# anovos/anovos

Measured on AMD Instinct MI355X. Metric: rows/sec (whole node) full analyzer+drift+transform, higher is better.
Workload: dtype fp32 data + fp64 accumulators; 1 GPU; model=anovos-full-pipeline, rows_per_gpu=125000000, n_cols=201, global_batch=125000000, parallelism=dp1

## Files before the change

### anovos_amd/ops/hip/anovos_kernels.hip

```cpp

#include <hip/hip_runtime.h>
#include <cfloat>
#include <cstdint>
#include <cmath>

#define THREADS 256
#define DEV_INLINE __device__ __forceinline__

typedef int nat_i4 __attribute__((ext_vector_type(4)));
typedef float nat_f4 __attribute__((ext_vector_type(4)));


#define NSTAT 9

struct MomAcc {
  double n, s1, s2, s3, s4, mn, mx, zn, nf;
};

DEV_INLINE void mom_add(MomAcc &a, double v, double shift) {
  if (!isnan(v)) {
    a.n += 1.0;
    double d = v - shift;
    a.s1 += d;
    double d2 = d * d;
    a.s2 += d2;
    a.s3 += d2 * d;
    a.s4 += d2 * d2;
    a.mn = fmin(a.mn, v);
    a.mx = fmax(a.mx, v);
    a.zn += (v == 0.0) ? 1.0 : 0.0;
    a.nf += (v != trunc(v)) ? 1.0 : 0.0;
  }
}

DEV_INLINE void mom_wave_reduce(MomAcc &a) {
  for (int off = 32; off > 0; off >>= 1) {
    a.n += __shfl_down(a.n, off);
    a.s1 += __shfl_down(a.s1, off);
    a.s2 += __shfl_down(a.s2, off);
    a.s3 += __shfl_down(a.s3, off);
    a.s4 += __shfl_down(a.s4, off);
    a.mn = fmin(a.mn, __shfl_down(a.mn, off));
    a.mx = fmax(a.mx, __shfl_down(a.mx, off));
    a.zn += __shfl_down(a.zn, off);
    a.nf += __shfl_down(a.nf, off);
  }
}

DEV_INLINE void mom_block_reduce_write(MomAcc &a, double *dst) {
  mom_wave_reduce(a);
  __shared__ double smw[(THREADS / 64) * NSTAT];
  const int wave = threadIdx.x >> 6;
  if ((threadIdx.x & 63) == 0) {
    double *m = &smw[wave * NSTAT];
    m[0] = a.n; m[1] = a.s1; m[2] = a.s2; m[3] = a.s3; m[4] = a.s4;
    m[5] = a.mn; m[6] = a.mx; m[7] = a.zn; m[8] = a.nf;
  }
  __syncthreads();
  if (threadIdx.x == 0) {
    MomAcc r{0, 0, 0, 0, 0, (double)INFINITY, -(double)INFINITY, 0, 0};
    for (int wv = 0; wv < THREADS / 64; ++wv) {
      double *m = &smw[wv * NSTAT];
      r.n += m[0]; r.s1 += m[1]; r.s2 += m[2]; r.s3 += m[3]; r.s4 += m[4];
      r.mn = fmin(r.mn, m[5]); r.mx = fmax(r.mx, m[6]);
      r.zn += m[7]; r.nf += m[8];
    }
    dst[0] = r.n; dst[1] = r.s1; dst[2] = r.s2; dst[3] = r.s3; dst[4] = r.s4;
    dst[5] = r.mn; dst[6] = r.mx; dst[7] = r.zn; dst[8] = r.nf;
  }
}

template <typename T>
__global__ __launch_bounds__(THREADS) void moments_partials_kernel(
    const T *const *cols, const int64_t *lens, const double *shifts, int nchunks,
    double *partials) {
  const int col = blockIdx.x / nchunks;
  const int chunk = blockIdx.x % nchunks;
  const T *__restrict__ x = cols[col];
  const int64_t n = lens[col];
  const double shift = shifts ? shifts[col] : 0.0;
  const int64_t per = (n + nchunks - 1) / nchunks;
  const int64_t s = (int64_t)chunk * per;
  const int64_t e = min(n, s + per);

  MomAcc a{0, 0, 0, 0, 0, (double)INFINITY, -(double)INFINITY, 0};

  if (sizeof(T) == 4) {
    const int64_t nv = (e - s) / 4;
    const float4 *xv = reinterpret_cast<const float4 *>(x + s);
    for (int64_t i = threadIdx.x; i < nv; i += THREADS) {
      float4 v = xv[i];
      mom_add(a, (double)v.x, shift);
      mom_add(a, (double)v.y, shift);
      mom_add(a, (double)v.z, shift);
      mom_add(a, (double)v.w, shift);
    }
    for (int64_t i = s + nv * 4 + threadIdx.x; i < e; i += THREADS) mom_add(a, (double)x[i], shift);
  } else {
    for (int64_t i = s + threadIdx.x; i < e; i += THREADS) mom_add(a, (double)x[i], shift);
  }

  mom_block_reduce_write(a, &partials[(int64_t)blockIdx.x * NSTAT]);
}

__global__ __launch_bounds__(THREADS) void moments_reduce_kernel(
    const double *partials, int nchunks, double *out) {
  const int col = blockIdx.x;
  MomAcc a{0, 0, 0, 0, 0, (double)INFINITY, -(double)INFINITY, 0, 0};
  for (int c = threadIdx.x; c < nchunks; c += THREADS) {
    const double *p = &partials[((int64_t)col * nchunks + c) * NSTAT];
    a.n += p[0]; a.s1 += p[1]; a.s2 += p[2]; a.s3 += p[3]; a.s4 += p[4];
    a.mn = fmin(a.mn, p[5]); a.mx = fmax(a.mx, p[6]); a.zn += p[7]; a.nf += p[8];
  }
  __shared__ double sm[THREADS * NSTAT];
  double *mine = &sm[threadIdx.x * NSTAT];
  mine[0] = a.n; mine[1] = a.s1; mine[2] = a.s2; mine[3] = a.s3;
  mine[4] = a.s4; mine[5] = a.mn; mine[6] = a.mx; mine[7] = a.zn; mine[8] = a.nf;
  __syncthreads();
  for (int stride = THREADS / 2; stride > 0; stride >>= 1) {
    if (threadIdx.x < stride) {
      double *other = &sm[(threadIdx.x + stride) * NSTAT];
      mine[0] += other[0]; mine[1] += other[1]; mine[2] += other[2];
      mine[3] += other[3]; mine[4] += other[4];
      mine[5] = fmin(mine[5], other[5]);
      mine[6] = fmax(mine[6], other[6]);
      mine[7] += other[7]; mine[8] += other[8];
    }
    __syncthreads();
  }
  if (threadIdx.x == 0) {
    double *o = &out[(int64_t)col * NSTAT];
    o[0] = sm[0]; o[1] = sm[1]; o[2] = sm[2]; o[3] = sm[3]; o[4] = sm[4];
    o[5] = (sm[0] > 0) ? sm[5] : nan("");
    o[6] = (sm[0] > 0) ? sm[6] : nan("");
    o[7] = sm[7]; o[8] = sm[8];
  }
}


template <typename T>
__global__ __launch_bounds__(THREADS) void hist_kernel(
    const T *const *cols, const int64_t *lens, const double *lo, const double *hi,
    int nbins, int nchunks, uint64_t *out ) {
  extern __shared__ uint32_t bins[];
  const int col = blockIdx.x / nchunks;
  const int chunk = blockIdx.x % nchunks;
  for (int b = threadIdx.x; b < nbins; b += THREADS) bins[b] = 0;
  __syncthreads();

  const T *__restrict__ x = cols[col];
  const int64_t n = lens[col];
  const int64_t per = (n + nchunks - 1) / nchunks;
  const int64_t s = (int64_t)chunk * per;
  const int64_t e = min(n, s + per);
  const double l = lo[col];
  const double h = hi[col];
  if (h > l) {
    const double scale = (double)nbins / (h - l);
    auto body = [&](double v) {
      if (!isnan(v)) {
        const double t = fmin(fmax((v - l) * scale, 0.0), (double)(nbins - 1));
        atomicAdd(&bins[(int)t], 1u);
      }
    };
    if (sizeof(T) == 4) {
      const int64_t nv = (e - s) / 4;
      const float4 *xv = reinterpret_cast<const float4 *>(x + s);
      for (int64_t i = threadIdx.x; i < nv; i += THREADS) {
        float4 v = xv[i];
        body((double)v.x);
        body((double)v.y);
        body((double)v.z);
        body((double)v.w);
      }
      for (int64_t i = s + nv * 4 + threadIdx.x; i < e; i += THREADS) body((double)x[i]);
    } else {
      for (int64_t i = s + threadIdx.x; i < e; i += THREADS) body((double)x[i]);
    }
  } else {
    for (int64_t i = s + threadIdx.x; i < e; i += THREADS) {
      double v = (double)x[i];
      if (!isnan(v)) atomicAdd(&bins[0], 1u);
    }
  }
  __syncthreads();
  uint64_t *g = &out[(int64_t)col * nbins];
  for (int b = threadIdx.x; b < nbins; b += THREADS)
    if (bins[b]) atomicAdd((unsigned long long *)&g[b], (unsigned long long)bins[b]);
}

template <typename T>
__global__ __launch_bounds__(THREADS) void bracket_hist_kernel(
    const T *const *cols, const int64_t *lens, const int64_t *colidx,
    const double *lo, const double *hi, int nbins, int nchunks, uint64_t *out) {
  extern __shared__ uint32_t bins[];
  const int bracket = blockIdx.x / nchunks;
  const int chunk = blockIdx.x % nchunks;
  for (int b = threadIdx.x; b < nbins; b += THREADS) bins[b] = 0;
  __syncthreads();
  const int col = (int)colidx[bracket];
  const T *__restrict__ x = cols[col];
  const int64_t n = lens[col];
  const int64_t per = (n + nchunks - 1) / nchunks;
  const int64_t s = (int64_t)chunk * per;
  const int64_t e = min(n, s + per);
  const double l = lo[bracket];
  const double h = hi[bracket];
  if (h > l) {
    const double scale = (double)nbins / (h - l);
    for (int64_t i = s + threadIdx.x; i < e; i += THREADS) {
      double v = (double)x[i];
      if (!isnan(v) && v >= l && v < h) {
        int b = (int)((v - l) * scale);
        b = max(0, min(nbins - 1, b));
        atomicAdd(&bins[b], 1u);
      }
    }
  }
  __syncthreads();
  uint64_t *g = &out[(int64_t)bracket * nbins];
  for (int b = threadIdx.x; b < nbins; b += THREADS)
    if (bins[b]) atomicAdd((unsigned long long *)&g[b], (unsigned long long)bins[b]);
}

#define RB_BINS 512
#define RB_MAXB 16

template <typename T>
__global__ __launch_bounds__(THREADS) void bracket_hist_grouped_kernel(
    const T *const *cols, const int64_t *lens, const int *bstart, int ncols,
    const double *lo, const double *hi, const double *p1lo,
    const double *p1scale, int p1bins, int nchunks, uint64_t *out) {
  __shared__ uint32_t bins[RB_MAXB * RB_BINS];
  extern __shared__ int16_t lut[];
  __shared__ double slo[RB_MAXB], sscale[RB_MAXB], shi[RB_MAXB];
  const int col = blockIdx.x / nchunks;
  const int chunk = blockIdx.x % nchunks;
  const int b0 = bstart[col];
  const int nb = bstart[col + 1] - b0;
  if (nb == 0) return;
  const double l1 = p1lo[col];
  const double sc1 = p1scale[col];
  for (int i = threadIdx.x; i < nb * RB_BINS; i += THREADS) bins[i] = 0;
  for (int i = threadIdx.x; i < p1bins; i += THREADS) lut[i] = -1;
  __syncthreads();
  if (threadIdx.x < nb) {
    const double bl = lo[b0 + threadIdx.x];
    const double bh = hi[b0 + threadIdx.x];
    slo[threadIdx.x] = bl;
    shi[threadIdx.x] = bh;
    double w = bh - bl;
    sscale[threadIdx.x] = (w > 0) ? (double)RB_BINS / w : 0.0;
    const double mid = (bl + bh) * 0.5;
    const int bin1 = (int)fmin(fmax((mid - l1) * sc1, 0.0), (double)(p1bins - 1));
// ... 245 lines not shown
}

__global__ __launch_bounds__(THREADS) void lut_apply_f32_kernel(
    const int32_t *const *cols, const int64_t *lens, const float *lutflat,
    const int64_t *lut_off, int nchunks, float *const *outs) {
  const int col = blockIdx.x / nchunks;
  const int chunk = blockIdx.x % nchunks;
  const int32_t *__restrict__ codes = cols[col];
  float *__restrict__ out = outs[col];
  const float *__restrict__ lut = &lutflat[lut_off[col]];
  const int64_t n = lens[col];
  const int64_t per = (n + nchunks - 1) / nchunks;
  const int64_t s = (int64_t)chunk * per;
  const int64_t e = min(n, s + per);
  const nat_i4 *__restrict__ cv = reinterpret_cast<const nat_i4 *>(codes + s);
  nat_f4 *__restrict__ ov = reinterpret_cast<nat_f4 *>(out + s);
  const int64_t nv = (e - s) / 4;
  for (int64_t i = threadIdx.x; i < nv; i += THREADS) {
    nat_i4 c = __builtin_nontemporal_load(&cv[i]);
    nat_f4 r;
    r.x = (c.x < 0) ? nanf("") : lut[c.x];
    r.y = (c.y < 0) ? nanf("") : lut[c.y];
    r.z = (c.z < 0) ? nanf("") : lut[c.z];
    r.w = (c.w < 0) ? nanf("") : lut[c.w];
    __builtin_nontemporal_store(r, &ov[i]);
  }
  for (int64_t j = s + nv * 4 + threadIdx.x; j < e; j += THREADS) {
    int c = codes[j];
    out[j] = (c < 0) ? nanf("") : lut[c];
  }
}

__global__ __launch_bounds__(THREADS) void lut_apply_i32_kernel(
    const int32_t *const *cols, const int64_t *lens, const int32_t *lutflat,
    const int64_t *lut_off, int nchunks, int32_t *const *outs) {
  const int col = blockIdx.x / nchunks;
  const int chunk = blockIdx.x % nchunks;
  const int32_t *__restrict__ codes = cols[col];
  int32_t *__restrict__ out = outs[col];
  const int32_t *__restrict__ lut = &lutflat[lut_off[col]];
  const int64_t n = lens[col];
  const int64_t per = (n + nchunks - 1) / nchunks;
  const int64_t s = (int64_t)chunk * per;
  const int64_t e = min(n, s + per);
  const nat_i4 *__restrict__ cv = reinterpret_cast<const nat_i4 *>(codes + s);
  nat_i4 *__restrict__ ov = reinterpret_cast<nat_i4 *>(out + s);
  const int64_t nv = (e - s) / 4;
  for (int64_t i = threadIdx.x; i < nv; i += THREADS) {
    nat_i4 c = __builtin_nontemporal_load(&cv[i]);
    nat_i4 r;
    r.x = (c.x < 0) ? -1 : lut[c.x];
    r.y = (c.y < 0) ? -1 : lut[c.y];
    r.z = (c.z < 0) ? -1 : lut[c.z];
    r.w = (c.w < 0) ? -1 : lut[c.w];
    __builtin_nontemporal_store(r, &ov[i]);
  }
  for (int64_t j = s + nv * 4 + threadIdx.x; j < e; j += THREADS) {
    int c = codes[j];
    out[j] = (c < 0) ? -1 : lut[c];
  }
}

__global__ __launch_bounds__(THREADS) void fill_code_kernel(
    const int32_t *const *cols, const int64_t *lens, const int32_t *fill,
    int nchunks, int32_t *const *outs) {
  const int col = blockIdx.x / nchunks;
  const int chunk = blockIdx.x % nchunks;
  const int32_t *__restrict__ x = cols[col];
  int32_t *__restrict__ out = outs[col];
  const int64_t n = lens[col];
  const int32_t fv = fill[col];
  const int64_t per = (n + nchunks - 1) / nchunks;
  const int64_t s = (int64_t)chunk * per;
  const int64_t e = min(n, s + per);
  const nat_i4 *__restrict__ xv = reinterpret_cast<const nat_i4 *>(x + s);
  nat_i4 *__restrict__ ov = reinterpret_cast<nat_i4 *>(out + s);
  const int64_t nv = (e - s) / 4;
  int64_t i = threadIdx.x;
  for (; i + THREADS < nv; i += 2 * THREADS) {
    nat_i4 a = __builtin_nontemporal_load(&xv[i]);
    nat_i4 b = __builtin_nontemporal_load(&xv[i + THREADS]);
    a.x = (a.x == -1) ? fv : a.x;
    a.y = (a.y == -1) ? fv : a.y;
    a.z = (a.z == -1) ? fv : a.z;
    a.w = (a.w == -1) ? fv : a.w;
    b.x = (b.x == -1) ? fv : b.x;
    b.y = (b.y == -1) ? fv : b.y;
    b.z = (b.z == -1) ? fv : b.z;
    b.w = (b.w == -1) ? fv : b.w;
    __builtin_nontemporal_store(a, &ov[i]);
    __builtin_nontemporal_store(b, &ov[i + THREADS]);
  }
  for (; i < nv; i += THREADS) {
    nat_i4 a = xv[i];
    a.x = (a.x == -1) ? fv : a.x;
    a.y = (a.y == -1) ? fv : a.y;
    a.z = (a.z == -1) ? fv : a.z;
    a.w = (a.w == -1) ? fv : a.w;
    ov[i] = a;
  }
  for (int64_t j = s + nv * 4 + threadIdx.x; j < e; j += THREADS) {
    int32_t c = x[j];
    out[j] = (c == -1) ? fv : c;
  }
}


__global__ __launch_bounds__(THREADS) void code_counts_kernel(
    const int32_t *codes, int64_t n, int size, int nchunks, uint64_t *out) {
  extern __shared__ uint32_t cnt[];
  const bool use_lds = (size <= 16384);
  if (use_lds) {
    for (int i = threadIdx.x; i < size; i += THREADS) cnt[i] = 0;
    __syncthreads();
  }
  const int chunk = blockIdx.x;
  const int64_t per = (n + nchunks - 1) / nchunks;
  const int64_t s = (int64_t)chunk * per;
  const int64_t e = min(n, s + per);
  if (use_lds) {
    for (int64_t i = s + threadIdx.x; i < e; i += THREADS) {
      int c = codes[i];
      if (c >= 0 && c < size) atomicAdd(&cnt[c], 1u);
    }
    __syncthreads();
    for (int i = threadIdx.x; i < size; i += THREADS)
      if (cnt[i]) atomicAdd((unsigned long long *)&out[i], (unsigned long long)cnt[i]);
  } else {
    for (int64_t i = s + threadIdx.x; i < e; i += THREADS) {
      int c = codes[i];
      if (c >= 0 && c < size) atomicAdd((unsigned long long *)&out[c], 1ull);
    }
  }
}


DEV_INLINE uint64_t splitmix64(uint64_t x) {
  x ^= x >> 30; x *= 0xBF58476D1CE4E5B9ull;
  x ^= x >> 27; x *= 0x94D049BB133111EBull;
  x ^= x >> 31;
  return x;
}

DEV_INLINE uint32_t fmix32(uint32_t x) {
  x ^= x >> 16;
  x *= 0x85EBCA6Bu;
  x ^= x >> 13;
  x *= 0xC2B2AE35u;
  x ^= x >> 16;
  return x;
}

template <typename T>
DEV_INLINE bool hll_hash(T v, int p, int &idx, int &rho) {
  if (sizeof(T) == 4) {
    float f = (float)v;
    if (isnan(f)) return false;
    uint32_t b32;
    memcpy(&b32, &f, 4);
    uint32_t h = fmix32(b32);
    idx = (int)(h >> (32 - p));
    uint32_t rem = h << p;
    rho = (rem == 0) ? (32 - p + 1) : (__clz((int)rem) + 1);
    if (rho > 32 - p + 1) rho = 32 - p + 1;
    return true;
  }
  double d = (double)v;
  if (isnan(d)) return false;
  uint64_t bits;
  memcpy(&bits, &d, 8);
  uint64_t h = splitmix64(bits);
  idx = (int)(h >> (64 - p));
  uint64_t rem = h << p;
  rho = (rem == 0) ? (64 - p + 1) : (__clzll((long long)rem) + 1);
  if (rho > 64 - p + 1) rho = 64 - p + 1;
  return true;
}

template <typename T>
__global__ __launch_bounds__(THREADS) void hll_kernel(
    const T *x, int64_t n, int p, int nchunks, int32_t *regs ) {
  extern __shared__ int32_t sreg[];
  const int m = 1 << p;
  for (int i = threadIdx.x; i < m; i += THREADS) sreg[i] = 0;
  __syncthreads();
  const int chunk = blockIdx.x;
  const int64_t per = (n + nchunks - 1) / nchunks;
  const int64_t s = (int64_t)chunk * per;
  const int64_t e = min(n, s + per);
  if (sizeof(T) == 4) {
    const float4 *xv = reinterpret_cast<const float4 *>(x + s);
    const int64_t nv = (e - s) / 4;
    for (int64_t i = threadIdx.x; i < nv; i += THREADS) {
      float4 v = xv[i];
      int idx, rho;
      if (hll_hash((T)v.x, p, idx, rho)) { if (sreg[idx] < rho) atomicMax(&sreg[idx], rho); }
      if (hll_hash((T)v.y, p, idx, rho)) { if (sreg[idx] < rho) atomicMax(&sreg[idx], rho); }
      if (hll_hash((T)v.z, p, idx, rho)) { if (sreg[idx] < rho) atomicMax(&sreg[idx], rho); }
      if (hll_hash((T)v.w, p, idx, rho)) { if (sreg[idx] < rho) atomicMax(&sreg[idx], rho); }
    }
    for (int64_t i = s + nv * 4 + threadIdx.x; i < e; i += THREADS) {
      int idx, rho;
      if (hll_hash(x[i], p, idx, rho)) { if (sreg[idx] < rho) atomicMax(&sreg[idx], rho); }
    }
  } else {
    for (int64_t i = s + threadIdx.x; i < e; i += THREADS) {
      int idx, rho;
      if (hll_hash(x[i], p, idx, rho)) { if (sreg[idx] < rho) atomicMax(&sreg[idx], rho); }
    }
  }
  __syncthreads();
  for (int i = threadIdx.x; i < m; i += THREADS)
    if (sreg[i]) atomicMax(&regs[i], sreg[i]);
}


#define ROWS_PB 8192
#define COLS_PB 64

DEV_INLINE bool is_null_elem(float v) { return isnan(v); }
DEV_INLINE bool is_null_elem(double v) { return isnan(v); }
DEV_INLINE bool is_null_elem(int32_t v) { return v == -1; }

template <typename T>
__global__ __launch_bounds__(THREADS) void row_null_kernel(
    const T *const *cols, int ncols, int64_t n, int32_t *out) {
  __shared__ uint16_t rc[ROWS_PB];
  const int ncolchunks = (ncols + COLS_PB - 1) / COLS_PB;
  const int rowchunk = blockIdx.x / ncolchunks;
  const int colchunk = blockIdx.x % ncolchunks;
  const int64_t s = (int64_t)rowchunk * ROWS_PB;
  const int64_t e = min(n, s + ROWS_PB);
  const int nr = (int)(e - s);
  const int c0 = colchunk * COLS_PB;
  const int c1 = min(ncols, c0 + COLS_PB);
  const bool vec_ok = (sizeof(T) == 4) && (nr % 4 == 0) && ((s & 3) == 0);
  if (vec_ok) {
    constexpr int QPT = ROWS_PB / 4 / THREADS;
    ushort4 acc[QPT];
#pragma unroll
    for (int q = 0; q < QPT; ++q) acc[q] = ushort4{0, 0, 0, 0};
    const int nq = nr / 4;
    typedef T T4 __attribute__((ext_vector_type(4)));
    for (int c = c0; c < c1; ++c) {
      const T4 *__restrict__ xv = reinterpret_cast<const T4 *>(cols[c] + s);
#pragma unroll
      for (int q = 0; q < QPT; ++q) {
        const int i = threadIdx.x + q * THREADS;
        if (i < nq) {
          T4 v = __builtin_nontemporal_load(&xv[i]);
          acc[q].x += is_null_elem((T)v.x);
          acc[q].y += is_null_elem((T)v.y);
          acc[q].z += is_null_elem((T)v.z);
          acc[q].w += is_null_elem((T)v.w);
        }
      }
    }
#pragma unroll
    for (int q = 0; q < QPT; ++q) {
      const int i = threadIdx.x + q * THREADS;
      if (i < nq) {
        const int64_t r = s + 4LL * i;
        if (ncolchunks == 1) {
          out[r] += (int32_t)acc[q].x;
          out[r + 1] += (int32_t)acc[q].y;
          out[r + 2] += (int32_t)acc[q].z;
          out[r + 3] += (int32_t)acc[q].w;
        } else {
          if (acc[q].x) atomicAdd(&out[r], (int32_t)acc[q].x);
          if (acc[q].y) atomicAdd(&out[r + 1], (int32_t)acc[q].y);
          if (acc[q].z) atomicAdd(&out[r + 2], (int32_t)acc[q].z);
          if (acc[q].w) atomicAdd(&out[r + 3], (int32_t)acc[q].w);
        }
      }
    }
    return;
  }
  for (int i = threadIdx.x; i < ROWS_PB / 4; i += THREADS)
    ((uint64_t *)rc)[i] = 0;
  __syncthreads();
  for (int c = c0; c < c1; ++c) {
    const T *__restrict__ x = cols[c] + s;
    for (int i = threadIdx.x; i < nr; i += THREADS)
      if (is_null_elem(x[i])) rc[i] += 1;
  }
  __syncthreads();
  if (ncolchunks == 1) {
    for (int i = threadIdx.x; i < nr; i += THREADS) out[s + i] += (int32_t)rc[i];
  } else {
    for (int i = threadIdx.x; i < nr; i += THREADS)
      if (rc[i]) atomicAdd(&out[s + i], (int32_t)rc[i]);
  }
}


template <typename T>
__global__ __launch_bounds__(THREADS) void hll_multi_kernel(
    const T *const *cols, const int64_t *lens, int p, int nchunks,
    int32_t *regs ) {
  extern __shared__ int32_t sreg[];
  const int m = 1 << p;
  const int col = blockIdx.x / nchunks;
  const int chunk = blockIdx.x % nchunks;
  for (int i = threadIdx.x; i < m; i += THREADS) sreg[i] = 0;
  __syncthreads();
  const T *__restrict__ x = cols[col];
  const int64_t n = lens[col];
  const int64_t per = (n + nchunks - 1) / nchunks;
  const int64_t s = (int64_t)chunk * per;
  const int64_t e = min(n, s + per);
  if (sizeof(T) == 4) {
    const float4 *xv = reinterpret_cast<const float4 *>(x + s);
    const int64_t nv = (e - s) / 4;
    for (int64_t i = threadIdx.x; i < nv; i += THREADS) {
      float4 v = xv[i];
      int idx, rho;
      if (hll_hash((T)v.x, p, idx, rho)) { if (sreg[idx] < rho) atomicMax(&sreg[idx], rho); }
      if (hll_hash((T)v.y, p, idx, rho)) { if (sreg[idx] < rho) atomicMax(&sreg[idx], rho); }
      if (hll_hash((T)v.z, p, idx, rho)) { if (sreg[idx] < rho) atomicMax(&sreg[idx], rho); }
      if (hll_hash((T)v.w, p, idx, rho)) { if (sreg[idx] < rho) atomicMax(&sreg[idx], rho); }
    }
    for (int64_t i = s + nv * 4 + threadIdx.x; i < e; i += THREADS) {
      int idx, rho;
      if (hll_hash(x[i], p, idx, rho)) { if (sreg[idx] < rho) atomicMax(&sreg[idx], rho); }
    }
  } else {
    for (int64_t i = s + threadIdx.x; i < e; i += THREADS) {
      int idx, rho;
// ... 371 lines not shown
    }
    __syncthreads();
    for (int i = threadIdx.x; i < slots; i += THREADS)
      if (cnt[i]) atomicAdd((unsigned long long *)&base[i], (unsigned long long)cnt[i]);
  } else {
    for (int64_t i = s + threadIdx.x; i < e; i += THREADS) {
      int c = codes[i];
      atomicAdd((unsigned long long *)&base[(c >= 0 && c < size) ? c : size], 1ull);
    }
  }
}

template <typename T>
__global__ __launch_bounds__(THREADS) void outlier_clamp_kernel(
    const T *const *cols, const int64_t *lens, const double *lo,
    const double *hi, int nchunks, int mode, T *const *outs,
    uint64_t *counts) {
  const int col = blockIdx.x / nchunks;
  const int chunk = blockIdx.x % nchunks;
  const T *__restrict__ x = cols[col];
  T *__restrict__ y = outs ? outs[col] : nullptr;
  const int64_t n = lens[col];
  const double l = lo[col], h = hi[col];
  const bool has_l = !isnan(l), has_h = !isnan(h);
  const int64_t per = (n + nchunks - 1) / nchunks;
  const int64_t s = (int64_t)chunk * per;
  const int64_t e = min(n, s + per);

  uint32_t nl = 0, nh = 0;
  const double lrep = (mode == 2) ? (double)NAN : l;
  const double hrep = (mode == 2) ? (double)NAN : h;
  auto clamp1 = [&](double v) -> double {
    const bool low = has_l && (v < l);
    const bool high = has_h && (v > h);
    nl += low ? 1u : 0u;
    nh += high ? 1u : 0u;
    if (mode) v = low ? lrep : (high ? hrep : v);
    return v;
  };
  if (sizeof(T) == 4) {
    float lf = (float)l;
    if ((double)lf < l) lf = nextafterf(lf, (float)INFINITY);
    float hf = (float)h;
    if ((double)hf > h) hf = nextafterf(hf, -(float)INFINITY);
    const float lrepf = (mode == 2) ? nanf("") : (float)l;
    const float hrepf = (mode == 2) ? nanf("") : (float)h;
    auto clamp1f = [&](float v) -> float {
      const bool low = has_l && (v < lf);
      const bool high = has_h && (v > hf);
      nl += low ? 1u : 0u;
      nh += high ? 1u : 0u;
      if (mode) v = low ? lrepf : (high ? hrepf : v);
      return v;
    };
    const nat_f4 *__restrict__ xv = reinterpret_cast<const nat_f4 *>(x + s);
    nat_f4 *__restrict__ ov = y ? reinterpret_cast<nat_f4 *>((float *)y + s) : nullptr;
    const int64_t nv = (e - s) / 4;
    int64_t i = threadIdx.x;
    for (; i + THREADS < nv; i += 2 * THREADS) {
      nat_f4 v = __builtin_nontemporal_load(&xv[i]);
      nat_f4 w = __builtin_nontemporal_load(&xv[i + THREADS]);
      v.x = clamp1f(v.x);
      v.y = clamp1f(v.y);
      v.z = clamp1f(v.z);
      v.w = clamp1f(v.w);
      w.x = clamp1f(w.x);
      w.y = clamp1f(w.y);
      w.z = clamp1f(w.z);
      w.w = clamp1f(w.w);
      if (mode && y) {
        __builtin_nontemporal_store(v, &ov[i]);
        __builtin_nontemporal_store(w, &ov[i + THREADS]);
      }
    }
    for (; i < nv; i += THREADS) {
      nat_f4 v = xv[i];
      v.x = clamp1f(v.x);
      v.y = clamp1f(v.y);
      v.z = clamp1f(v.z);
      v.w = clamp1f(v.w);
      if (mode && y) ov[i] = v;
    }
    for (int64_t j = s + nv * 4 + threadIdx.x; j < e; j += THREADS) {
      float v = clamp1f((float)x[j]);
      if (mode && y) y[j] = (T)v;
    }
  } else {
    for (int64_t i = s + threadIdx.x; i < e; i += THREADS) {
      double v = clamp1((double)x[i]);
      if (mode && y) y[i] = (T)v;
    }
  }
  __shared__ uint32_t red[2][THREADS];
  red[0][threadIdx.x] = nl;
  red[1][threadIdx.x] = nh;
  __syncthreads();
  for (int st = THREADS / 2; st > 0; st >>= 1) {
    if (threadIdx.x < st) {
      red[0][threadIdx.x] += red[0][threadIdx.x + st];
      red[1][threadIdx.x] += red[1][threadIdx.x + st];
    }
    __syncthreads();
  }
  if (threadIdx.x == 0) {
    if (red[0][0]) atomicAdd((unsigned long long *)&counts[col * 2 + 0], (unsigned long long)red[0][0]);
    if (red[1][0]) atomicAdd((unsigned long long *)&counts[col * 2 + 1], (unsigned long long)red[1][0]);
  }
}

extern "C" {

int anovos_code_counts_multi(const int32_t *const *cols, const int64_t *lens,
                             const int64_t *offs, const int *sizes, int ncols,
                             int lds_slots, int nchunks, uint64_t *out,
                             hipStream_t stream) {
  if (lds_slots < 0 || lds_slots > 16384) return (int)hipErrorInvalidValue;
  size_t lds = (size_t)lds_slots * 4;
  hipLaunchKernelGGL(code_counts_multi_kernel, dim3(ncols * nchunks),
                     dim3(THREADS), lds, stream, cols, lens, offs, sizes,
                     nchunks, out);
  return (int)hipGetLastError();
}

int anovos_outlier_clamp(const void *const *cols, const int64_t *lens,
                         int ncols, const double *lo, const double *hi,
                         int nchunks, int mode, int dtype, void *const *outs,
                         uint64_t *counts, hipStream_t stream) {
  if (dtype == 0)
    hipLaunchKernelGGL(outlier_clamp_kernel<float>, dim3(ncols * nchunks),
                       dim3(THREADS), 0, stream, (const float *const *)cols,
                       lens, lo, hi, nchunks, mode, (float *const *)outs,
                       counts);
  else
    hipLaunchKernelGGL(outlier_clamp_kernel<double>, dim3(ncols * nchunks),
                       dim3(THREADS), 0, stream, (const double *const *)cols,
                       lens, lo, hi, nchunks, mode, (double *const *)outs,
                       counts);
  return (int)hipGetLastError();
}

}

template <typename T>
__global__ __launch_bounds__(THREADS) void moments_hll_kernel(
    const T *const *cols, const int64_t *lens, const double *shifts, int p,
    int nchunks, double *partials, int32_t *regs ) {
  extern __shared__ int32_t sreg[];
  const int m = 1 << p;
  const int col = blockIdx.x / nchunks;
  const int chunk = blockIdx.x % nchunks;
  for (int i = threadIdx.x; i < m; i += THREADS) sreg[i] = 0;
  __syncthreads();

  const T *__restrict__ x = cols[col];
  const int64_t n = lens[col];
  const double shift = shifts ? shifts[col] : 0.0;
  const int64_t per = (n + nchunks - 1) / nchunks;
  const int64_t s = (int64_t)chunk * per;
  const int64_t e = min(n, s + per);

  MomAcc a{0, 0, 0, 0, 0, (double)INFINITY, -(double)INFINITY, 0};
  auto body = [&](T v) {
    mom_add(a, (double)v, shift);
    int idx, rho;
    if (hll_hash(v, p, idx, rho)) { if (sreg[idx] < rho) atomicMax(&sreg[idx], rho); }
  };
  if (sizeof(T) == 4) {
    const int64_t nv = (e - s) / 4;
    const float4 *xv = reinterpret_cast<const float4 *>(x + s);
    for (int64_t i = threadIdx.x; i < nv; i += THREADS) {
      float4 v = xv[i];
      body((T)v.x);
      body((T)v.y);
      body((T)v.z);
      body((T)v.w);
    }
    for (int64_t i = s + nv * 4 + threadIdx.x; i < e; i += THREADS) body(x[i]);
  } else {
    for (int64_t i = s + threadIdx.x; i < e; i += THREADS) body(x[i]);
  }

  mom_block_reduce_write(a, &partials[(int64_t)blockIdx.x * NSTAT]);
  int32_t *g = &regs[(int64_t)col * m];
  for (int i = threadIdx.x; i < m; i += THREADS)
    if (sreg[i]) atomicMax(&g[i], sreg[i]);
}

extern "C" int anovos_moments_hll(const void *const *cols, const int64_t *lens,
                                  const double *shifts, int ncols, int p,
                                  int nchunks, int dtype, double *partials,
                                  double *mom_out, int32_t *regs,
                                  hipStream_t stream) {
  dim3 grid(ncols * nchunks);
  size_t lds = (size_t)(1 << p) * 4;
  if (dtype == 0)
    hipLaunchKernelGGL(moments_hll_kernel<float>, grid, dim3(THREADS), lds, stream,
                       (const float *const *)cols, lens, shifts, p, nchunks, partials, regs);
  else
    hipLaunchKernelGGL(moments_hll_kernel<double>, grid, dim3(THREADS), lds, stream,
                       (const double *const *)cols, lens, shifts, p, nchunks, partials, regs);
  hipLaunchKernelGGL(moments_reduce_kernel, dim3(ncols), dim3(THREADS), 0, stream,
                     partials, nchunks, mom_out);
  return (int)hipGetLastError();
}

DEV_INLINE int label_slot_f32(float v, int slots) {
  if (v != v) return 0;
  const int slot = (int)fminf(fmaxf(v, -1.0f), (float)(slots - 1)) + 1;
  return (slot >= slots) ? slots - 1 : slot;
}

__global__ __launch_bounds__(THREADS) void label_counts_multi_kernel(
    const void *const *cols, const uint8_t *__restrict__ label,
    const int64_t *lens, const int64_t *offs, const int *sizes,
    const int *dtypes, int nchunks, uint64_t *out) {
  const int col = blockIdx.x / nchunks;
  const int chunk = blockIdx.x % nchunks;
  const int slots = sizes[col];
  uint64_t *base = out + offs[col];
  extern __shared__ uint32_t lds2[];
  uint32_t *tot = lds2;
  uint32_t *evt = lds2 + slots;
  for (int i = threadIdx.x; i < 2 * slots; i += THREADS) lds2[i] = 0;
  __syncthreads();
  const int64_t n = lens[col];
  const int64_t per = (n + nchunks - 1) / nchunks;
  const int64_t s = (int64_t)chunk * per;
  const int64_t e = min(n, s + per);
  if (dtypes[col] == 0) {
    const float *__restrict__ x = (const float *)cols[col];
    const int64_t nv = (e - s) / 4;
    const nat_f4 *__restrict__ xv = reinterpret_cast<const nat_f4 *>(x + s);
    for (int64_t i = threadIdx.x; i < nv; i += THREADS) {
      nat_f4 v = __builtin_nontemporal_load(&xv[i]);
      const int64_t r = s + i * 4;
      float vv[4] = {v.x, v.y, v.z, v.w};
#pragma unroll
      for (int k = 0; k < 4; ++k) {
        const int slot = label_slot_f32(vv[k], slots);
        atomicAdd(&tot[slot], 1u);
        if (label[r + k]) atomicAdd(&evt[slot], 1u);
      }
    }
    for (int64_t i = s + nv * 4 + threadIdx.x; i < e; i += THREADS) {
      const int slot = label_slot_f32(x[i], slots);
      atomicAdd(&tot[slot], 1u);
      if (label[i]) atomicAdd(&evt[slot], 1u);
    }
  } else {
    const int32_t *__restrict__ codes = (const int32_t *)cols[col];
    const int64_t nv = (e - s) / 4;
    const nat_i4 *__restrict__ cv = reinterpret_cast<const nat_i4 *>(codes + s);
    for (int64_t i = threadIdx.x; i < nv; i += THREADS) {
      nat_i4 c = __builtin_nontemporal_load(&cv[i]);
      const int64_t r = s + i * 4;
      int cc[4] = {c.x, c.y, c.z, c.w};
#pragma unroll
      for (int k = 0; k < 4; ++k) {
        int slot = (cc[k] >= 0 && cc[k] < slots - 1) ? cc[k] : slots - 1;
        atomicAdd(&tot[slot], 1u);
        if (label[r + k]) atomicAdd(&evt[slot], 1u);
      }
    }
    for (int64_t i = s + nv * 4 + threadIdx.x; i < e; i += THREADS) {
      int c = codes[i];
      int slot = (c >= 0 && c < slots - 1) ? c : slots - 1;
      atomicAdd(&tot[slot], 1u);
      if (label[i]) atomicAdd(&evt[slot], 1u);
    }
  }
  __syncthreads();
  for (int i = threadIdx.x; i < slots; i += THREADS) {
    if (tot[i]) atomicAdd((unsigned long long *)&base[i], (unsigned long long)tot[i]);
    if (evt[i]) atomicAdd((unsigned long long *)&base[slots + i], (unsigned long long)evt[i]);
  }
}

extern "C" int anovos_label_counts_multi(
    const void *const *cols, const uint8_t *label, const int64_t *lens,
    const int64_t *offs, const int *sizes, const int *dtypes, int ncols,
    int max_slots, int nchunks, uint64_t *out, hipStream_t stream) {
  size_t lds = (size_t)max_slots * 2 * sizeof(uint32_t);
  hipLaunchKernelGGL(label_counts_multi_kernel, dim3(ncols * nchunks),
                     dim3(THREADS), lds, stream, cols, label, lens, offs,
                     sizes, dtypes, nchunks, out);
  return (int)hipGetLastError();
}

template <typename T, int NREG>
__global__ __launch_bounds__(THREADS) void bucketize_label_counts_kernel(
    const T *const *cols, const uint8_t *__restrict__ label,
    const int64_t *lens, const double *cutflat, const int64_t *cutoff_off,
    const int *cutoff_len, const int64_t *offs, const int *sizes,
    int max_ncut, int max_slots, int nchunks, uint64_t *out) {
  extern __shared__ double smem[];
  const int col = blockIdx.x / nchunks;
  const int chunk = blockIdx.x % nchunks;
  const int ncut = cutoff_len[col];
  const int slots = sizes[col];
  double *cuts = smem;
  float *cutsf = reinterpret_cast<float *>(cuts);
  uint32_t *cnt = reinterpret_cast<uint32_t *>(smem + max_ncut);
  uint32_t *tot = cnt;
  uint32_t *evt = cnt + slots;
  const double *src = &cutflat[cutoff_off[col]];
  if (sizeof(T) == 4) {
    for (int i = threadIdx.x; i < ncut; i += THREADS) {
      double c = src[i];
      float cf = (float)c;
      if ((double)cf > c) cf = nextafterf(cf, -(float)INFINITY);
      cutsf[i] = cf;
    }
  } else {
    for (int i = threadIdx.x; i < ncut; i += THREADS) cuts[i] = src[i];
  }
  for (int i = threadIdx.x; i < 2 * slots; i += THREADS) cnt[i] = 0;
  __syncthreads();
  RegCuts<NREG> rc;
  if (NREG > 0) rc.load(cutsf, ncut);

  const T *__restrict__ x = cols[col];
  const int64_t n = lens[col];
  const int64_t per = (n + nchunks - 1) / nchunks;
  const int64_t s = (int64_t)chunk * per;
  const int64_t e = min(n, s + per);

  auto slot_f32 = [&](float v) -> int {
    if (v != v) return 0;
    int lo = 0;
    if (NREG > 0) {
      lo = rc.below(v);
    } else if (ncut <= 32) {
      for (int j = 0; j < ncut; ++j) lo += (cutsf[j] < v) ? 1 : 0;
    } else {
// ... 145 lines not shown
```

Measured before the change: 438.8 million rows/sec.

## Stream moments/HLL inputs with prefetched nontemporal loads and wave-ballot counters

Moments and fused moments+HLL kernels now read columns through a register double-buffered, nontemporal global load loop. Counts (n, zeros, non-integers) are computed per wave with ballot+popcount into integer counters. Min/max are kept in the native type, and HLL rho uses a branchless clz with a sentinel bit. Register-array HLL lookups are batched per float4. The goal is to cut fp64 work and branches per element and hide load latency, at the cost of more registers and a changed non-integer test (abs comparison).

```diff
diff --git a/anovos_amd/ops/hip/anovos_kernels.hip b/anovos_amd/ops/hip/anovos_kernels.hip
--- a/anovos_amd/ops/hip/anovos_kernels.hip
+++ b/anovos_amd/ops/hip/anovos_kernels.hip
@@ -10,6 +10,38 @@
 typedef int nat_i4 __attribute__((ext_vector_type(4)));
 typedef float nat_f4 __attribute__((ext_vector_type(4)));
 
+template <typename T>
+using gptr = T __attribute__((address_space(1))) *;
+template <typename T>
+DEV_INLINE gptr<T> to_global(T *p) {
+  return (gptr<T>)p;
+}
+
+#define STREAM_U 2
+template <typename E, typename F>
+DEV_INLINE void stream_prefetched(gptr<const E> xv, int64_t nv, F &&f) {
+  const int64_t ntrips = nv / (STREAM_U * THREADS);
+  gptr<const E> p = xv + threadIdx.x;
+  if (ntrips > 0) {
+    E cur[STREAM_U], nxt[STREAM_U];
+#pragma unroll
+    for (int u = 0; u < STREAM_U; ++u) cur[u] = __builtin_nontemporal_load(p + u * THREADS);
+    for (int64_t it = 1; it < ntrips; ++it) {
+      p += STREAM_U * THREADS;
+#pragma unroll
+      for (int u = 0; u < STREAM_U; ++u) nxt[u] = __builtin_nontemporal_load(p + u * THREADS);
+#pragma unroll
+      for (int u = 0; u < STREAM_U; ++u) f(cur[u]);
+#pragma unroll
+      for (int u = 0; u < STREAM_U; ++u) cur[u] = nxt[u];
+    }
+#pragma unroll
+    for (int u = 0; u < STREAM_U; ++u) f(cur[u]);
+  }
+  for (int64_t i = ntrips * (STREAM_U * THREADS) + threadIdx.x; i < nv; i += THREADS)
+    f(__builtin_nontemporal_load(xv + i));
+}
+
 
 #define NSTAT 9
 
@@ -17,21 +49,47 @@
   double n, s1, s2, s3, s4, mn, mx, zn, nf;
 };
 
-DEV_INLINE void mom_add(MomAcc &a, double v, double shift) {
-  if (!isnan(v)) {
-    a.n += 1.0;
-    double d = v - shift;
-    a.s1 += d;
+DEV_INLINE float trunc_t(float v) { return truncf(v); }
+DEV_INLINE double trunc_t(double v) { return trunc(v); }
+DEV_INLINE float abs_t(float v) { return fabsf(v); }
+DEV_INLINE double abs_t(double v) { return fabs(v); }
+DEV_INLINE float min_t(float a, float b) { return fminf(a, b); }
+DEV_INLINE double min_t(double a, double b) { return fmin(a, b); }
+DEV_INLINE float max_t(float a, float b) { return fmaxf(a, b); }
+DEV_INLINE double max_t(double a, double b) { return fmax(a, b); }
+
+template <typename T>
+struct MomLane {
+  double s1 = 0, s2 = 0, s3 = 0, s4 = 0;
+  T mn = (T)INFINITY, mx = -(T)INFINITY;
+  uint64_t n = 0, zn = 0, nf = 0;
+  DEV_INLINE void add(T v, double shift) {
+    double d = (double)v - shift;
+    s1 += d;
     double d2 = d * d;
-    a.s2 += d2;
-    a.s3 += d2 * d;
-    a.s4 += d2 * d2;
-    a.mn = fmin(a.mn, v);
-    a.mx = fmax(a.mx, v);
-    a.zn += (v == 0.0) ? 1.0 : 0.0;
-    a.nf += (v != trunc(v)) ? 1.0 : 0.0;
-  }
-}
+    s2 += d2;
+    s3 += d2 * d;
+    s4 += d2 * d2;
+  }
+  DEV_INLINE void count(T v) {
+    n += __popcll(__ballot(v == v));
+    zn += __popcll(__ballot(v == (T)0));
+    nf += __popcll(__ballot(abs_t(v) > abs_t(trunc_t(v))));
+  }
+  DEV_INLINE void minmax(T v) {
+    mn = min_t(mn, v);
+    mx = max_t(mx, v);
+  }
+  DEV_INLINE void minmax4(T a, T b, T c, T d) {
+    mn = min_t(min_t(min_t(min_t(mn, a), b), c), d);
+    mx = max_t(max_t(max_t(max_t(mx, a), b), c), d);
+  }
+  DEV_INLINE MomAcc acc() const {
+    const bool lead = (threadIdx.x & 63) == 0;
+    return MomAcc{lead ? (double)n : 0.0, s1, s2, s3, s4, (double)mn, (double)mx,
+                  lead ? (double)zn : 0.0, lead ? (double)nf : 0.0};
+  }
+};
 
 DEV_INLINE void mom_wave_reduce(MomAcc &a) {
   for (int off = 32; off > 0; off >>= 1) {
@@ -76,30 +134,36 @@
     double *partials) {
   const int col = blockIdx.x / nchunks;
   const int chunk = blockIdx.x % nchunks;
-  const T *__restrict__ x = cols[col];
+  const gptr<const T> x = to_global(cols[col]);
   const int64_t n = lens[col];
   const double shift = shifts ? shifts[col] : 0.0;
   const int64_t per = (n + nchunks - 1) / nchunks;
   const int64_t s = (int64_t)chunk * per;
   const int64_t e = min(n, s + per);
 
-  MomAcc a{0, 0, 0, 0, 0, (double)INFINITY, -(double)INFINITY, 0};
-
+  MomLane<T> lane;
+  auto body = [&](T v) {
+    lane.count(v);
+    lane.minmax(v);
+    if (v == v) lane.add(v, shift);
+  };
   if (sizeof(T) == 4) {
     const int64_t nv = (e - s) / 4;
-    const float4 *xv = reinterpret_cast<const float4 *>(x + s);
-    for (int64_t i = threadIdx.x; i < nv; i += THREADS) {
-      float4 v = xv[i];
-      mom_add(a, (double)v.x, shift);
-      mom_add(a, (double)v.y, shift);
-      mom_add(a, (double)v.z, shift);
-      mom_add(a, (double)v.w, shift);
-    }
-    for (int64_t i = s + nv * 4 + threadIdx.x; i < e; i += THREADS) mom_add(a, (double)x[i], shift);
+    stream_prefetched<nat_f4>((gptr<const nat_f4>)(x + s), nv, [&](nat_f4 q) {
+      const T v[4] = {(T)q.x, (T)q.y, (T)q.z, (T)q.w};
+      lane.minmax4(v[0], v[1], v[2], v[3]);
+#pragma unroll
+      for (int k = 0; k < 4; ++k) {
+        lane.count(v[k]);
+        if (v[k] == v[k]) lane.add(v[k], shift);
+      }
+    });
+    for (int64_t i = s + nv * 4 + threadIdx.x; i < e; i += THREADS) body(x[i]);
   } else {
-    for (int64_t i = s + threadIdx.x; i < e; i += THREADS) mom_add(a, (double)x[i], shift);
-  }
-
+    stream_prefetched<T>(x + s, e - s, body);
+  }
+
+  MomAcc a = lane.acc();
   mom_block_reduce_write(a, &partials[(int64_t)blockIdx.x * NSTAT]);
 }
 
@@ -651,28 +715,28 @@
 }
 
 template <typename T>
-DEV_INLINE bool hll_hash(T v, int p, int &idx, int &rho) {
+DEV_INLINE void hll_idx_rho(T v, int p, int &idx, int &rho) {
   if (sizeof(T) == 4) {
     float f = (float)v;
-    if (isnan(f)) return false;
     uint32_t b32;
     memcpy(&b32, &f, 4);
     uint32_t h = fmix32(b32);
     idx = (int)(h >> (32 - p));
-    uint32_t rem = h << p;
-    rho = (rem == 0) ? (32 - p + 1) : (__clz((int)rem) + 1);
-    if (rho > 32 - p + 1) rho = 32 - p + 1;
-    return true;
+    rho = __clz((int)((h << p) | (1u << (p - 1)))) + 1;
+    return;
   }
   double d = (double)v;
-  if (isnan(d)) return false;
   uint64_t bits;
   memcpy(&bits, &d, 8);
   uint64_t h = splitmix64(bits);
   idx = (int)(h >> (64 - p));
-  uint64_t rem = h << p;
-  rho = (rem == 0) ? (64 - p + 1) : (__clzll((long long)rem) + 1);
-  if (rho > 64 - p + 1) rho = 64 - p + 1;
+  rho = __clzll((long long)((h << p) | (1ull << (p - 1)))) + 1;
+}
+
+template <typename T>
+DEV_INLINE bool hll_hash(T v, int p, int &idx, int &rho) {
+  if (v != v) return false;
+  hll_idx_rho(v, p, idx, rho);
   return true;
 }
 
@@ -1350,34 +1414,49 @@
   for (int i = threadIdx.x; i < m; i += THREADS) sreg[i] = 0;
   __syncthreads();
 
-  const T *__restrict__ x = cols[col];
+  const gptr<const T> __restrict__ x = to_global(cols[col]);
   const int64_t n = lens[col];
   const double shift = shifts ? shifts[col] : 0.0;
   const int64_t per = (n + nchunks - 1) / nchunks;
   const int64_t s = (int64_t)chunk * per;
   const int64_t e = min(n, s + per);
 
-  MomAcc a{0, 0, 0, 0, 0, (double)INFINITY, -(double)INFINITY, 0};
+  MomLane<T> lane;
   auto body = [&](T v) {
-    mom_add(a, (double)v, shift);
-    int idx, rho;
-    if (hll_hash(v, p, idx, rho)) { if (sreg[idx] < rho) atomicMax(&sreg[idx], rho); }
+    lane.count(v);
+    lane.minmax(v);
+    if (v == v) {
+      lane.add(v, shift);
+      int idx, rho;
+      hll_idx_rho(v, p, idx, rho);
+      if (sreg[idx] < rho) atomicMax(&sreg[idx], rho);
+    }
   };
   if (sizeof(T) == 4) {
     const int64_t nv = (e - s) / 4;
-    const float4 *xv = reinterpret_cast<const float4 *>(x + s);
-    for (int64_t i = threadIdx.x; i < nv; i += THREADS) {
-      float4 v = xv[i];
-      body((T)v.x);
-      body((T)v.y);
-      body((T)v.z);
-      body((T)v.w);
-    }
+    stream_prefetched<nat_f4>((gptr<const nat_f4>)(x + s), nv, [&](nat_f4 q) {
+      const T v[4] = {(T)q.x, (T)q.y, (T)q.z, (T)q.w};
+      int idx[4], rho[4], cur[4];
+#pragma unroll
+      for (int k = 0; k < 4; ++k) hll_idx_rho(v[k], p, idx[k], rho[k]);
+#pragma unroll
+      for (int k = 0; k < 4; ++k) cur[k] = sreg[idx[k]];
+      lane.minmax4(v[0], v[1], v[2], v[3]);
+#pragma unroll
+      for (int k = 0; k < 4; ++k) {
+        lane.count(v[k]);
+        if (v[k] == v[k]) {
+          lane.add(v[k], shift);
+          if (cur[k] < rho[k]) atomicMax(&sreg[idx[k]], rho[k]);
+        }
+      }
+    });
     for (int64_t i = s + nv * 4 + threadIdx.x; i < e; i += THREADS) body(x[i]);
   } else {
-    for (int64_t i = s + threadIdx.x; i < e; i += THREADS) body(x[i]);
-  }
-
+    stream_prefetched<T>(x + s, e - s, body);
+  }
+
+  MomAcc a = lane.acc();
   mom_block_reduce_write(a, &partials[(int64_t)blockIdx.x * NSTAT]);
   int32_t *g = &regs[(int64_t)col * m];
   for (int i = threadIdx.x; i < m; i += THREADS)
```

Result: slower. 426.7 million rows/sec (-2.8%).
